# zju3dv/LoFTR

Hardware: AMD Instinct MI355X
Metric: image-pairs/sec @640x480 indoor-ds (higher is better)
Workload: dtype f32; 1 GPU; batch=8 640x480 synthetic grayscale pairs per GPU, indoor_ds dual-softmax (BASELINE configs[1]), full LoFTR.forward = ResNet-FPN backbone (HIP implicit-GEMM / patch convolutions incl. the 7x7 stem) + HIP matching path; weights=seeded random init (no checkpoint on the box), conf_matrix_materialised=True, match_type=dual_softmax, global_batch=8, parallelism=dp1 (pairs sharded; RCCL all-gather of match counts)

## Files before the change

loftr_amd/csrc/common.h:

```cpp
#pragma once
#include <hip/hip_runtime.h>
#include <stdint.h>
#include <stddef.h>
#include "../../include/loftr_hip.h"

typedef float f32x16 __attribute__((ext_vector_type(16)));
typedef float f32x4 __attribute__((ext_vector_type(4)));
typedef float f32x2 __attribute__((ext_vector_type(2)));

#define LOFTR_NEG_INF (-1e9f)

#define LOFTR_CHECK_ARG(cond) do { if (!(cond)) return LOFTR_ERR_BAD_ARG; } while (0)
#define LOFTR_CHECK_LAUNCH() do { if (hipGetLastError() != hipSuccess) return LOFTR_ERR_LAUNCH; } while (0)

#ifdef __HIP_DEVICE_COMPILE__
#define LOFTR_NO_PACKED_FP32 __attribute__((target("no-packed-fp32-ops")))
#else
#define LOFTR_NO_PACKED_FP32
#endif

__host__ __device__ static inline int ceil_div(int a, int b) { return (a + b - 1) / b; }
static inline size_t align_up(size_t x, size_t a) { return (x + a - 1) / a * a; }

enum LoftrTimedKernel {
  LOFTR_T_SCORE_STATS = 0,
  LOFTR_T_SCORE_CONF = 1,
  LOFTR_T_PROJ = 2,
  LOFTR_T_LINEAR = 3,
  LOFTR_T_LINEAR_LN = 4,
  LOFTR_T_KV = 5,
  LOFTR_T_ATTN_APPLY = 6,
  LOFTR_T_ATTN_SMALL = 7,
  LOFTR_T_GATHER = 8,
  LOFTR_T_OT_STORE = 9,
  LOFTR_T_CONV = 10,
  LOFTR_T_CONV3 = 11,
  LOFTR_T_CONV3W = 12,
  LOFTR_T_ENCODER_X = 13,
  LOFTR_T_FINE_PAIR = 14,
  LOFTR_T_COUNT = 15
};
enum LoftrDebugKey {
  LOFTR_DBG_ENCODER_SCHEDULE = 0,
  LOFTR_DBG_CONV_PERSIST_CAP,
  LOFTR_DBG_WGRAD_CHUNK,
  LOFTR_DBG_REDUCE_TALL,
  LOFTR_DBG_PCT_GRID,
  LOFTR_DBG_PCT_SKIP,
  LOFTR_DBG_PCT_QUOTA,
  LOFTR_DBG_CONV_DUO,
  LOFTR_DBG_CONV_PATCH,
  LOFTR_DBG_CONV_REM,
  LOFTR_DBG_FINE_WAVES,
  LOFTR_DBG_COUNT
};
int loftr_debug_value(int key);
extern unsigned g_loftr_timing_mask;
extern int g_loftr_range_check;
void loftr_timing_mark(int id, hipStream_t st, bool end);
struct TimedLaunch {
  int id; hipStream_t st; bool on;
  TimedLaunch(int id_, hipStream_t st_) : id(id_), st(st_), on((g_loftr_timing_mask >> id_) & 1u) {
    if (on) loftr_timing_mark(id, st, false);
  }
  ~TimedLaunch() { if (on) loftr_timing_mark(id, st, true); }
};

constexpr int NUM_XCD = 8;
static inline unsigned xcd_grid(int tiles_m, int tiles_n) { return (unsigned)(NUM_XCD * ceil_div(tiles_m, NUM_XCD) * tiles_n); }
__device__ __forceinline__ bool xcd_tile(int tiles_m, int tiles_n, int& tile_m, int& tile_n) {
  const int id = blockIdx.x, xcd = id % NUM_XCD, slot = id / NUM_XCD;
  const int chunk = ceil_div(tiles_m, NUM_XCD);
  tile_n = slot % tiles_n;
  const int local = slot / tiles_n;
  tile_m = xcd * chunk + local;
  return local < chunk && tile_m < tiles_m;
}

struct WsAlloc {
  char* base; size_t cap; size_t off;
  WsAlloc(void* p, size_t bytes) : base((char*)p), cap(bytes), off(0) {}
  template <typename T> T* take(size_t n) {
    off = align_up(off, 256);
    T* r = (T*)(base + off);
    off += n * sizeof(T);
    return r;
  }
  bool ok() const { return off <= cap; }
};

__device__ __forceinline__ float wave_sum(float v) {
#pragma unroll
  for (int o = 32; o >= 1; o >>= 1) v += __shfl_xor(v, o, 64);
  return v;
}
__device__ __forceinline__ float wave_max(float v) {
#pragma unroll
  for (int o = 32; o >= 1; o >>= 1) v = fmaxf(v, __shfl_xor(v, o, 64));
  return v;
}
#define LOFTR_DPP(v_, ctrl_) __int_as_float(__builtin_amdgcn_update_dpp(0, __float_as_int(v_), ctrl_, 0xF, 0xF, true))
#define LOFTR_DPPI(v_, ctrl_) __builtin_amdgcn_update_dpp(0, v_, ctrl_, 0xF, 0xF, true)
__device__ __forceinline__ float half_sum(float v) {
  v += LOFTR_DPP(v, 0xB1);
  v += LOFTR_DPP(v, 0x4E);
  v += LOFTR_DPP(v, 0x141);
  v += LOFTR_DPP(v, 0x140);
  const auto r = __builtin_amdgcn_permlane16_swap(__float_as_int(v), __float_as_int(v), false, false);
  return __int_as_float(r[0]) + __int_as_float(r[1]);
}
__device__ __forceinline__ float half_max(float v) {
  v = fmaxf(v, LOFTR_DPP(v, 0xB1));
  v = fmaxf(v, LOFTR_DPP(v, 0x4E));
  v = fmaxf(v, LOFTR_DPP(v, 0x141));
  v = fmaxf(v, LOFTR_DPP(v, 0x140));
  const auto r = __builtin_amdgcn_permlane16_swap(__float_as_int(v), __float_as_int(v), false, false);
  return fmaxf(__int_as_float(r[0]), __int_as_float(r[1]));
}
__device__ __forceinline__ int half_min_i32(int v) {
  v = min(v, LOFTR_DPPI(v, 0xB1));
  v = min(v, LOFTR_DPPI(v, 0x4E));
  v = min(v, LOFTR_DPPI(v, 0x141));
  v = min(v, LOFTR_DPPI(v, 0x140));
  const auto r = __builtin_amdgcn_permlane16_swap(v, v, false, false);
  return min((int)r[0], (int)r[1]);
}
__device__ __forceinline__ void half_sum16(f32x16& v) {
#pragma unroll
  for (int r = 0; r < 16; ++r) v[r] += LOFTR_DPP(v[r], 0xB1);
#pragma unroll
  for (int r = 0; r < 16; ++r) v[r] += LOFTR_DPP(v[r], 0x4E);
#pragma unroll
  for (int r = 0; r < 16; ++r) v[r] += LOFTR_DPP(v[r], 0x141);
#pragma unroll
  for (int r = 0; r < 16; ++r) v[r] += LOFTR_DPP(v[r], 0x140);
#pragma unroll
  for (int r = 0; r < 16; ++r) {
    const auto q = __builtin_amdgcn_permlane16_swap(__float_as_int(v[r]), __float_as_int(v[r]), false, false);
    v[r] = __int_as_float(q[0]) + __int_as_float(q[1]);
  }
}
__device__ __forceinline__ void half_max16(f32x16& v) {
#pragma unroll
  for (int r = 0; r < 16; ++r) v[r] = fmaxf(v[r], LOFTR_DPP(v[r], 0xB1));
#pragma unroll
  for (int r = 0; r < 16; ++r) v[r] = fmaxf(v[r], LOFTR_DPP(v[r], 0x4E));
#pragma unroll
  for (int r = 0; r < 16; ++r) v[r] = fmaxf(v[r], LOFTR_DPP(v[r], 0x141));
#pragma unroll
  for (int r = 0; r < 16; ++r) v[r] = fmaxf(v[r], LOFTR_DPP(v[r], 0x140));
#pragma unroll
  for (int r = 0; r < 16; ++r) {
    const auto q = __builtin_amdgcn_permlane16_swap(__float_as_int(v[r]), __float_as_int(v[r]), false, false);
    v[r] = fmaxf(__int_as_float(q[0]), __int_as_float(q[1]));
  }
}
__device__ __forceinline__ float swap32(float v) {
  const auto r = __builtin_amdgcn_permlane32_swap(__float_as_int(v), __float_as_int(v), false, false);
  return __int_as_float((threadIdx.x & 32) ? r[0] : r[1]);
}
#define LOFTR_DPP_SWAP32(v_) swap32(v_)

__device__ __forceinline__ float elu1(float x) {
  return x > 0.f ? x + 1.f : __expf(x);
}
```

loftr_amd/csrc/conv.hip:

```cpp
#include "gemm.h"
#include "conv_prepared.h"
#include <stdlib.h>

namespace {

using CfgD = GemmCfg<256, 128, 4, 2, 3>;

struct ConvArgs {
  ASrc a;
  const sp_t* w; int K;
  const float* bias;
  const float* wscale;
  const float* x_inv;
  const sp_t* residual;
  sp_t* y_sp;
  float* y_f32;
  int M, Cout, Coutp;
  int act;
  const sp_t* up;
  int Hl, Wl;
  float sy, sx;
};

template <typename Cfg, bool FULL>
// ... 266 lines not shown
        acc[i][j] = __builtin_amdgcn_mfma_f32_32x32x16_f16(fh[(R0_) + i][ks_], bl[ks_][j], acc[i][j], 0, 0, 0); \
    _Pragma("unroll") for (int i = 0; i < 2; ++i)                                                           \
      _Pragma("unroll") for (int j = 0; j < (NJ_); ++j)                                                     \
        acc[i][j] = __builtin_amdgcn_mfma_f32_32x32x16_f16(fh[(R0_) + i][ks_], bh[ks_][j], acc[i][j], 0, 0, 0); \
  }
#define C3_PIN_PAIRS(n_)                                                                                    \
    _Pragma("unroll") for (int u__ = 0; u__ < (n_); ++u__) {                                                \
      __builtin_amdgcn_sched_group_barrier(0x008, 1, 0);                                                    \
      __builtin_amdgcn_sched_group_barrier(0x100, 1, 0);                                                    \
    }
#define C3_ITER(KY, NJ_, DEAD_)                                                                             \
  {                                                                                                         \
    const int tt__ = t + (KY);                                                                              \
     \
    const int newer__ = (tt__ + 2 < nk ? 2 : 0) + ((patch_m1 || patch_m2) ? PQ : 0);                        \
    if (newer__ >= 2 + PQ) LOFTR_WAITCNT_VM(2 + PQ);                                                        \
    else if (newer__ >= PQ) LOFTR_WAITCNT_VM(PQ);                                                           \
    else if (newer__ >= 2) LOFTR_WAITCNT_VM(2);                                                             \
    else LOFTR_WAITCNT_VM(0);                                                                               \
    __builtin_amdgcn_s_barrier();                                                                           \
    if (tt__ + 3 < nk) C3_ISSUE_B(cg3, (q3 % 3) * 3 + q3 / 3, (bstage + 3) & 3);                            \
    if (++q3 == 9) { q3 = 0; ++cg3; }                                                                       \
    patch_m2 = patch_m1;                                                                                    \
    patch_m1 = false;                                                                                       \
    if ((KY) == 0 && kx == 0 && cg + 1 < gpt) { C3_ISSUE_PATCH(cg + 1, (cg + 1) & 1); patch_m1 = true; }    \
    if ((NJ_) > 0) {                                                                                        \
      constexpr int n1__ = ((KY) == 0 ? 4 : 2) + 2 * (NJ_);                 \
      constexpr int n0__ = ((KY) == 2 ? 4 : 2) + 2 * (NJ_);             \
      if (!(DEAD_)) {                                                                                       \
        if ((KY) == 0) { C3_LOAD_ROW(0, 1, sP, kx); C3_LOAD_ROW(1, 1, sP, kx); }                            \
        else C3_LOAD_ROW((KY) + 1, 1, sP, kx);                                                              \
        C3_LOAD_B(1, bstage, NJ_);                                                                          \
      }                                                                                                     \
      C3_MFMAS(0, KY, NJ_);                                                                                 \
                                         \
      if ((KY) == 2) { C3_LOAD_ROW(0, 0, sPn, kxn); C3_LOAD_ROW(1, 0, sPn, kxn); }                          \
      else C3_LOAD_ROW((KY) + 2, 0, sP, kx);                                                                \
      C3_LOAD_B(0, (bstage + 1) & 3, NJ_);                                                                  \
      if (!(DEAD_)) C3_MFMAS(1, KY, NJ_);                                                                   \
                            \
      if (!(DEAD_)) {                                                                                       \
        C3_PIN_PAIRS(n1__) __builtin_amdgcn_sched_group_barrier(0x008, 6 * (NJ_) - n1__, 0);                \
      }                                                                                                     \
      C3_PIN_PAIRS(n0__) __builtin_amdgcn_sched_group_barrier(0x008, 6 * (NJ_) - n0__, 0);                  \
    }                                                                                                       \
    bstage = (bstage + 1) & 3;                                                                              \
  }
#define C3_TRIP(NJ_, DEAD_)                                                                                 \
  {                                                                                                         \
    const char* sP = patch_base + (cg & 1) * PATCH_BYTES;                                                   \
    const int kxn = kx == 2 ? 0 : kx + 1;                           \
    const char* sPn = patch_base + ((cg + (kx == 2 ? 1 : 0)) & 1) * PATCH_BYTES;                            \
    C3_ITER(0, NJ_, DEAD_)                                                                                  \
    C3_ITER(1, NJ_, DEAD_)                                                                                  \
    C3_ITER(2, NJ_, DEAD_)                                                                                  \
    if (++kx == 3) { kx = 0; ++cg; }                                                                        \
  }
  const bool dead_last = p.Cin <= (gpt - 1) * 32 + 16;
#define C3_LOOP(NJ_)                                                                                        \
  {                                                                                                         \
     \
    LOFTR_WAITCNT_VM(4);                                                                                    \
    __builtin_amdgcn_s_barrier();                                                                           \
    if ((NJ_) > 0) {                                                                                        \
      C3_LOAD_ROW(0, 0, patch_base, 0);                                                                     \
      C3_LOAD_ROW(1, 0, patch_base, 0);                                                                     \
      C3_LOAD_B(0, 0, NJ_);                                                                                 \
    }                                                                                                       \
    int t = 0;                                                                                              \
    for (; t < nk - 9; t += 3) C3_TRIP(NJ_, 0)                                                              \
    if (dead_last) { for (; t < nk; t += 3) C3_TRIP(NJ_, 1) }                                               \
    else { for (; t < nk; t += 3) C3_TRIP(NJ_, 0) }                                                         \
  }
  if (nact == 2) C3_LOOP(2)
  else if (nact == 1) C3_LOOP(1)
  else C3_LOOP(0)
#undef C3_LOOP
#undef C3_TRIP
#undef C3_ITER
#undef C3_PIN_PAIRS
#undef C3_MFMAS
#undef C3_LOAD_B
#undef C3_LOAD_ROW

  vid += gridDim.x;
  C3_NEXT_TILE()
  __builtin_amdgcn_s_barrier();
  if (have) {
    C3_DMA_OFFSETS()
    C3_ISSUE_PATCH(0, 0);
    C3_ISSUE_B(0, 0, 0);
    C3_ISSUE_B(0, 3, 1);
    C3_ISSUE_B(0, 6, 2);
  }

  const bool odd = lane & 1;
  const int Ho = p.H, Wo = p.W;
#pragma unroll
  for (int j = 0; j < 2; ++j) {
    const int col = n0 + wn * 64 + j * 32 + tx;
    const bool creal = col < p.Cout, cpad = col < p.Coutp;
    const float bia = (p.bias && creal) ? p.bias[col] : 0.f;
    const float wsc = (creal ? p.wscale[col] : 1.f) * (p.x_inv ? *p.x_inv : 1.f);
    const int spc = (col & ~31) + (odd ? 16 : 0) + ((col & 31) >> 1);
#pragma unroll
    for (int i = 0; i < 2; ++i) {
      const int y = y0 + wm * 2 + i;
      f32x16 v = acc[i][j] * wsc;
      uint32_t rw[16];
      if (p.residual) {
#pragma unroll
        for (int r = 0; r < 16; ++r) {
          const int x = x0 + (r & 3) + 8 * (r >> 2) + 4 * g;
          const bool ok = y < Ho && x < Wo && cpad;
          rw[r] = ok ? p.residual[(unsigned)(((b * Ho + y) * Wo + x) * p.Coutp + spc)] : 0u;
        }
#pragma unroll
        for (int r = 0; r < 16; ++r) v[r] += sp_value(rw[r], odd);
      }
#pragma unroll
      for (int r = 0; r < 16; ++r) {
        float xv = v[r] + bia;
        if (p.act == 1) xv = fmaxf(xv, 0.f);
        if (p.act == 2) xv = xv > 0.f ? xv : 0.01f * xv;
        v[r] = creal ? xv : 0.f;
      }
      if (p.y_f32) {
#pragma unroll
        for (int r = 0; r < 16; ++r) {
          const int x = x0 + (r & 3) + 8 * (r >> 2) + 4 * g;
          if (y < Ho && x < Wo && creal) p.y_f32[(unsigned)(((b * Ho + y) * Wo + x) * p.Cout + col)] = v[r];
        }
      }
      if (p.y_sp) {
        uint32_t w16[16];
        sp_words16(v, odd, w16);
#pragma unroll
        for (int r = 0; r < 16; ++r) {
          const int x = x0 + (r & 3) + 8 * (r >> 2) + 4 * g;
          if (y < Ho && x < Wo && cpad) p.y_sp[(unsigned)(((b * Ho + y) * Wo + x) * p.Coutp + spc)] = w16[r];
        }
      }
    }
  }
  if (!have) break;
  }
#undef C3_ISSUE_PATCH
#undef C3_ISSUE_B
#undef C3_DMA_OFFSETS
#undef C3_NEXT_TILE
}

#include "conv3x3_duo.h"


__global__ __launch_bounds__(256) void conv_rowscale_kernel(const float* __restrict__ w, const float* __restrict__ bn_w,
                                                            const float* __restrict__ bn_b, const float* __restrict__ bn_m,
                                                            const float* __restrict__ bn_v, float eps, int Cin, int KH, int KW,
                                                            long s_co, long s_ci, long s_ky, long s_kx,
                                                            float* __restrict__ bias, float* __restrict__ wscale) {
  const int co = blockIdx.x;
  float scale = 1.f, shift = 0.f;
  if (bn_w) {
    scale = bn_w[co] / sqrtf(bn_v[co] + eps);
    shift = bn_b[co] - bn_m[co] * scale;
  }
  float m = 0.f;
  for (int t = threadIdx.x; t < Cin * KH * KW; t += 256) {
    const int c = t % Cin, tap = t / Cin;
    m = fmaxf(m, fabsf(w[co * s_co + c * s_ci + (tap / KW) * s_ky + (tap % KW) * s_kx] * scale));
  }
  __shared__ float red[4];
  m = wave_max(m);
  if ((threadIdx.x & 63) == 0) red[threadIdx.x >> 6] = m;
  __syncthreads();
  if (threadIdx.x == 0) {
    float inv;
    (void)sp_row_scale(fmaxf(fmaxf(red[0], red[1]), fmaxf(red[2], red[3])), &inv);
    bias[co] = shift;
    wscale[co] = inv;
  }
}

__global__ __launch_bounds__(256) void conv_prep_kernel(const float* __restrict__ w, const float* __restrict__ bn_w,
                                                        const float* __restrict__ bn_b, const float* __restrict__ bn_m,
                                                        const float* __restrict__ bn_v, float eps, int Cin, int Cp,
                                                        int KH, int KW, long s_co, long s_ci, long s_ky, long s_kx,
                                                        sp_t* __restrict__ wsp, const float* __restrict__ wscale) {
  const int co = blockIdx.y;
  const int K = KH * KW * Cp;
  float scale = 1.f;
  if (bn_w) scale = bn_w[co] / sqrtf(bn_v[co] + eps);
  const float up = 1.f / wscale[co];
  const int grp = blockIdx.x * 8 + (threadIdx.x >> 5);
  if (grp * 32 >= K) return;
  const int col = grp * 32 + (threadIdx.x & 31);
  const int tap = col / Cp, c = col - tap * Cp;
  float v = 0.f;
  if (c < Cin) v = (w[co * s_co + c * s_ci + (tap / KW) * s_ky + (tap % KW) * s_kx] * scale) * up;
  sp_store(wsp + (long)co * K, col, v, true);
}

__global__ __launch_bounds__(256) void upsample_add_kernel(const sp_t* __restrict__ low, const sp_t* __restrict__ lat,
                                                           sp_t* __restrict__ out, int Hl, int Wl, int Cp, long nitems) {
  const long item = (long)blockIdx.x * 256 + threadIdx.x;
  if (item >= nitems) return;
  const int octs = Cp >> 3;
  const long pix = item / octs;
  const int oct = (int)(item - pix * octs);
  const int Ho = 2 * Hl, Wo = 2 * Wl;
  const int x = (int)(pix % Wo), y = (int)((pix / Wo) % Ho);
  const long b = pix / ((long)Wo * Ho);
  const float sy = Ho > 1 ? (float)(Hl - 1) / (float)(Ho - 1) : 0.f, sx = Wo > 1 ? (float)(Wl - 1) / (float)(Wo - 1) : 0.f;
  const float fy = sy * (float)y, fx = sx * (float)x;
  const int y0 = (int)fy, x0 = (int)fx;
  const int y1 = y0 + (y0 < Hl - 1 ? 1 : 0), x1 = x0 + (x0 < Wl - 1 ? 1 : 0);
  const float ly = fy - (float)y0, lx = fx - (float)x0;
  const float hy = 1.f - ly, hx = 1.f - lx;
  const int off = sp_octet_off(oct);
  const sp_t* src[5] = {low + ((b * Hl + y0) * Wl + x0) * Cp + off, low + ((b * Hl + y0) * Wl + x1) * Cp + off,
                        low + ((b * Hl + y1) * Wl + x0) * Cp + off, low + ((b * Hl + y1) * Wl + x1) * Cp + off,
                        lat + pix * Cp + off};
  u32x4 hi[5], lo[5];
#pragma unroll
  for (int t = 0; t < 5; ++t) {
    hi[t] = *reinterpret_cast<const u32x4*>(src[t]);
    lo[t] = *reinterpret_cast<const u32x4*>(src[t] + 16);
  }
  float v[5][8];
#pragma unroll
  for (int t = 0; t < 5; ++t) sp_unpack8(hi[t], lo[t], v[t]);
  float r[8];
#pragma unroll
  for (int e = 0; e < 8; ++e)
    r[e] = v[4][e] + (hy * (hx * v[0][e] + lx * v[1][e]) + ly * (hx * v[2][e] + lx * v[3][e]));
  u32x4 oh, ol;
  sp_pack8(r, oh, ol);
  sp_t* o = out + pix * Cp + off;
  *reinterpret_cast<u32x4*>(o) = oh;
  *reinterpret_cast<u32x4*>(o + 16) = ol;
}

constexpr int STEM_TY = 8, STEM_TX = 32;
__global__ __launch_bounds__(256) void stem_conv_kernel(const float* __restrict__ x, long sxb, long sxh, long sxw,
                                                        int H, int W, const float* __restrict__ w, long s_co, long s_ky,
                                                        long s_kx, const float* __restrict__ bn_w,
                                                        const float* __restrict__ bn_b, const float* __restrict__ bn_m,
                                                        const float* __restrict__ bn_v, float eps, int C0, int Ho, int Wo,
                                                        sp_t* __restrict__ y) {
  constexpr int IH = 2 * STEM_TY + 5, IW = 2 * STEM_TX + 5;
  __shared__ float tile[IH][IW + 3];
  const int b = blockIdx.z, oy0 = blockIdx.y * STEM_TY, ox0 = blockIdx.x * STEM_TX;
  const float* xb = x + (long)b * sxb;
  for (int e = threadIdx.x; e < IH * IW; e += 256) {
    const int r = e / IW, c = e - r * IW;
    const int iy = 2 * oy0 - 3 + r, ix = 2 * ox0 - 3 + c;
    tile[r][c] = ((unsigned)iy < (unsigned)H && (unsigned)ix < (unsigned)W) ? xb[iy * sxh + ix * sxw] : 0.f;
  }
  const int ch = threadIdx.x & 127, slot = threadIdx.x >> 7;
  float wr[49];
  float scale = 1.f, shift = 0.f;
  if (ch < C0) {
    if (bn_w) { scale = bn_w[ch] / sqrtf(bn_v[ch] + eps); shift = bn_b[ch] - bn_m[ch] * scale; }
#pragma unroll
    for (int t = 0; t < 49; ++t) wr[t] = w[ch * s_co + (t / 7) * s_ky + (t % 7) * s_kx] * scale;
  } else {
#pragma unroll
    for (int t = 0; t < 49; ++t) wr[t] = 0.f;
  }
  __syncthreads();
  const int Cp = (C0 + 31) / 32 * 32;
  for (int q = slot; q < STEM_TY * STEM_TX / 4; q += 2) {
    const int py = q / (STEM_TX / 4), px = (q - py * (STEM_TX / 4)) * 4;
    float acc[4] = {shift, shift, shift, shift};
#pragma unroll
    for (int ky = 0; ky < 7; ++ky) {
      float row[13];
#pragma unroll
      for (int c = 0; c < 13; ++c) row[c] = tile[2 * py + ky][2 * px + c];
#pragma unroll
      for (int kx = 0; kx < 7; ++kx)
#pragma unroll
        for (int e = 0; e < 4; ++e) acc[e] += row[2 * e + kx] * wr[ky * 7 + kx];
    }
    const int oy = oy0 + py;
#pragma unroll
    for (int e = 0; e < 4; ++e) {
      const int ox = ox0 + px + e;
      const float v = fmaxf(acc[e], 0.f);
      const bool ok = oy < Ho && ox < Wo && ch < Cp;
      const uint32_t word = sp_word(ch < C0 ? v : 0.f, ch & 1);
      if (ok) y[(((long)b * Ho + oy) * Wo + ox) * Cp + sp_index(ch)] = word;
    }
  }
}

__global__ void sp_to_f32_kernel(const sp_t* __restrict__ src, float* __restrict__ dst, long rows, int C, int Cp) {
  const long row = blockIdx.x;
  for (int c = threadIdx.x; c < Cp; c += blockDim.x) {
    const float v = sp_value(src[row * Cp + sp_index(c)], c & 1);
    if (c < C) dst[row * C + c] = v;
  }
}

}

extern "C" size_t loftr_conv_workspace_bytes(int Cin, int Cout, int KH, int KW) {
  if (Cin <= 0 || Cout <= 0 || KH <= 0 || KW <= 0) return 0;
  return align_up((size_t)Cout * KH * KW * ceil32(Cin) * 4, 256) + 2 * align_up((size_t)Cout * 4, 256) + 2048;
}

static unsigned persistent_grid(unsigned nvirt) {
  const int cap = loftr_debug_value(LOFTR_DBG_CONV_PERSIST_CAP);
  const int forced = cap >= NUM_XCD ? cap / NUM_XCD * NUM_XCD : -1;
  int cus = forced;
  if (cus < 0) {
    static int per_dev[64];
    int dev = 0, n = 0;
    if (hipGetDevice(&dev) != hipSuccess || dev < 0 || dev >= 64) return nvirt;
    if (per_dev[dev] == 0) {
      if (hipDeviceGetAttribute(&n, hipDeviceAttributeMultiprocessorCount, dev) != hipSuccess) return nvirt;
      per_dev[dev] = n / NUM_XCD * NUM_XCD;
    }
    cus = per_dev[dev];
  }
  return cus > 0 && nvirt > (unsigned)cus ? (unsigned)cus : nvirt;
}

template <int RT>
__global__ __launch_bounds__(256) void conv_rem_gather_kernel(const float* __restrict__ pbuf, long npix, int H, int W, int R, int c0, int Coutp,
                                                              const float* __restrict__ bias, const sp_t* __restrict__ residual, int act,
                                                              sp_t* __restrict__ y_sp) {
  const long pix = (long)blockIdx.x * 256 + threadIdx.x;
  if (pix >= npix) return;
  const int x = (int)(pix % W), y = (int)((pix / W) % H);
  float v[8];
#pragma unroll
  for (int c = 0; c < 8; ++c) v[c] = 0.f;
  const float* pp = pbuf + pix * (9 * R);
#pragma unroll
  for (int ky = 0; ky < 3; ++ky)
#pragma unroll
    for (int kx = 0; kx < 3; ++kx) {
      const int yy = y + ky - 1, xx = x + kx - 1;
      if ((unsigned)yy < (unsigned)H && (unsigned)xx < (unsigned)W) {
        const float* q = pp + ((long)(ky - 1) * W + (kx - 1)) * (9 * R) + (ky * 3 + kx) * R;
        if (RT == 4) {
          const f32x4 t = *reinterpret_cast<const f32x4*>(q);
          v[0] += t[0]; v[1] += t[1]; v[2] += t[2]; v[3] += t[3];
        } else {
#pragma unroll
          for (int c = 0; c < 7; ++c) if (c < R) v[c] += q[c];
        }
      }
    }
  sp_t* row = y_sp + pix * Coutp + c0;
  float rv[8];
#pragma unroll
  for (int c = 0; c < 8; ++c) rv[c] = 0.f;
  if (residual) {
    const sp_t* rr = residual + pix * Coutp + c0;
    const u32x4 hi = *reinterpret_cast<const u32x4*>(rr), lo = *reinterpret_cast<const u32x4*>(rr + 16);
    sp_unpack8(hi, lo, rv);
  }
  const float slope = act == 1 ? 0.f : act == 2 ? 0.01f : 1.f;
  float o[8];
#pragma unroll
  for (int c = 0; c < 8; ++c) {
    const float t = v[c] + ((bias && c < R) ? bias[c0 + c] : 0.f) + rv[c];
    o[c] = c < R ? fmaxf(t, slope * t) : 0.f;
  }
  u32x4 oh, ol;
  sp_pack8(o, oh, ol);
  const u32x4 z = {0u, 0u, 0u, 0u};
  u32x4* dst = reinterpret_cast<u32x4*>(row);
  dst[0] = oh; dst[1] = z; dst[2] = z; dst[3] = z; dst[4] = ol; dst[5] = z; dst[6] = z; dst[7] = z;
}


static int conv_prepare(const float* weight, const long* weight_strides, int Cin, int Cout, int KH, int KW,
                        const float* bn_weight, const float* bn_bias, const float* bn_mean, const float* bn_var, float bn_eps,
                        void* buf, size_t bytes, hipStream_t st) {
  LOFTR_CHECK_ARG(weight && weight_strides && buf && Cin > 0 && Cout > 0 && KH > 0 && KW > 0);
  LOFTR_CHECK_ARG((bn_weight == nullptr) == (bn_bias == nullptr) && (bn_weight == nullptr) == (bn_mean == nullptr) &&
                  (bn_weight == nullptr) == (bn_var == nullptr));
  ConvPrepared pr;
  if (!conv_prepared_layout(buf, bytes, Cin, Cout, KH, KW, pr)) return LOFTR_ERR_WORKSPACE;
  const int Cp = ceil32(Cin), K = KH * KW * Cp;
  (void)hipMemsetAsync(pr.zeros, 0, 256, st);
  hipLaunchKernelGGL(conv_rowscale_kernel, dim3(Cout), dim3(256), 0, st, weight, bn_weight, bn_bias, bn_mean, bn_var, bn_eps,
                     Cin, KH, KW, weight_strides[0], weight_strides[1], weight_strides[2], weight_strides[3], pr.bias, pr.wscale);
  hipLaunchKernelGGL(conv_prep_kernel, dim3(ceil_div(K / 32, 8), Cout), dim3(256), 0, st, weight, bn_weight, bn_bias,
                     bn_mean, bn_var, bn_eps, Cin, Cp, KH, KW, weight_strides[0], weight_strides[1], weight_strides[2],
                     weight_strides[3], pr.wsp, pr.wscale);
  LOFTR_CHECK_LAUNCH();
  return LOFTR_OK;
}

static int conv_rem_channels(int Cout, int KH, int KW, int stride) {
  return (KH == 3 && KW == 3 && stride == 1 && ceil32(Cout) == 224 && Cout - 192 >= 1 && Cout - 192 <= 7) ? Cout - 192 : 0;
}
extern "C" size_t loftr_conv_scratch_bytes(int B, int H, int W, int Cout, int KH, int KW, int stride) {
  const int R = conv_rem_channels(Cout, KH, KW, stride);
  return (R > 0 && B > 0 && H > 0 && W > 0) ? (size_t)B * H * W * 9 * R * 4 : 0;
}

static int conv_run(const uint32_t* x_sp, int B, int H, int W, int Cin, const void* prepared, size_t prepared_bytes, int Cout,
                    int KH, int KW, int stride, int pad, int act, const uint32_t* residual_sp, const uint32_t* up_sp,
                    uint32_t* y_sp, float* y_f32, void* stream, const float* x_inv = nullptr, void* scratch = nullptr, size_t scratch_bytes = 0) {
  LOFTR_CHECK_ARG(x_sp && prepared && (y_sp || y_f32) && B >= 0 && H > 0 && W > 0 && Cin > 0 && Cout > 0);
  const bool shared_gpu = (act & LOFTR_CONV_SHARED_GPU) != 0;
  act &= ~LOFTR_CONV_SHARED_GPU;
  LOFTR_CHECK_ARG(KH > 0 && KW > 0 && stride > 0 && pad >= 0 && act >= 0 && act <= 2);
  if (B == 0) return LOFTR_OK;
  hipStream_t st = (hipStream_t)stream;
  ConvGeom g;
  g.H = H; g.W = W; g.Cp = ceil32(Cin); g.KH = KH; g.KW = KW; g.stride = stride; g.pad = pad;
  g.Ho = (H + 2 * pad - KH) / stride + 1;
  g.Wo = (W + 2 * pad - KW) / stride + 1;
  if (g.Ho <= 0 || g.Wo <= 0 || H >= 32768 || W >= 32768) return LOFTR_ERR_UNSUPPORTED;
  if (up_sp && ((g.Ho & 1) || (g.Wo & 1) || KH != 1 || KW != 1 || stride != 1 || pad != 0 || !y_sp || y_f32 || residual_sp || act != 0))
    return LOFTR_ERR_UNSUPPORTED;
  const long M = (long)B * g.Ho * g.Wo;
  if (M * (long)ceil32(Cout) >= (1L << 31) || (long)B * H * W * g.Cp >= (1L << 31)) return LOFTR_ERR_UNSUPPORTED;
  const int K = KH * KW * g.Cp;
  ConvPrepared pr;
  if (!conv_prepared_layout(const_cast<void*>(prepared), prepared_bytes, Cin, Cout, KH, KW, pr)) return LOFTR_ERR_WORKSPACE;
  sp_t* wsp = pr.wsp;
  float* bias = pr.bias;
  sp_t* zeros = pr.zeros;
  g.zeros = zeros;
  ConvArgs p;
  p.a = asrc_conv(x_sp, g);
  p.w = wsp; p.K = K; p.bias = bias; p.wscale = pr.wscale; p.x_inv = x_inv; p.residual = residual_sp; p.y_sp = y_sp; p.y_f32 = y_f32;
  p.M = (int)M; p.Cout = Cout; p.Coutp = ceil32(Cout); p.act = act;
  p.up = up_sp; p.Hl = g.Ho / 2; p.Wl = g.Wo / 2;
  p.sy = g.Ho > 1 ? (float)(p.Hl - 1) / (float)(g.Ho - 1) : 0.f;
  p.sx = g.Wo > 1 ? (float)(p.Wl - 1) / (float)(g.Wo - 1) : 0.f;
  if (loftr_debug_value(LOFTR_DBG_CONV_PATCH) && KH == 3 && KW == 3 && stride == 1 && pad == 1 && !up_sp) {
    Conv3Args c;
    c.x = x_sp; c.B = B; c.H = H; c.W = W; c.Cp = g.Cp; c.Cin = Cin; c.w = wsp; c.K = K; c.bias = bias; c.wscale = pr.wscale; c.x_inv = x_inv; c.residual = residual_sp;
    c.y_sp = y_sp; c.y_f32 = y_f32; c.Cout = Cout; c.Coutp = ceil32(Cout); c.act = act; c.zeros = zeros;
    c.tiles_x = ceil_div(W, c3::TX); c.tiles_y = ceil_div(H, c3::TY); c.pbuf = nullptr;
    const bool duo = loftr_debug_value(LOFTR_DBG_CONV_DUO) != 0;
    const bool wide = duo && c.Coutp == 32 * 7;
    TimedLaunch tl(wide ? LOFTR_T_CONV3W : LOFTR_T_CONV3, st);
    if (duo && c.Coutp % 128 == 0) {
      using CF = c3d::Cfg<4, 2, 4>;
      c.tiles_y = ceil_div(H, CF::TY);
      hipLaunchKernelGGL((conv3x3_duo_kernel<CF>), dim3(xcd_grid(B * c.tiles_x * c.tiles_y, c.Coutp / 128)), dim3(256), 0, st, c);
    } else if (duo && c.Coutp == 192) {
      using CF = c3d::Cfg<6, 2, 4, 8, 2>;
      c.tiles_y = ceil_div(H, CF::TY);
      hipLaunchKernelGGL((conv3x3_duo_kernel<CF>), dim3(xcd_grid(B * c.tiles_x * c.tiles_y, 1)), dim3(512), 0, st, c);
    } else if (wide && conv_rem_channels(Cout, KH, KW, stride) > 0 && !y_f32 && loftr_debug_value(LOFTR_DBG_CONV_REM) &&
               scratch && scratch_bytes >= (size_t)B * H * W * 9 * conv_rem_channels(Cout, KH, KW, stride) * 4) {
      using CF = c3d::Cfg<6, 2, 4, 8, 2, true>;
      c.tiles_y = ceil_div(H, CF::TY);
      c.pbuf = reinterpret_cast<float*>(scratch);
      hipLaunchKernelGGL((conv3x3_duo_kernel<CF>), dim3(xcd_grid(B * c.tiles_x * c.tiles_y, 1)), dim3(512), 0, st, c);
      LOFTR_CHECK_LAUNCH();
      const long npix = (long)B * H * W;
      if (Cout - 192 == 4)
        hipLaunchKernelGGL(conv_rem_gather_kernel<4>, dim3((unsigned)((npix + 255) / 256)), dim3(256), 0, st, c.pbuf, npix, H, W, 4, 192, c.Coutp,
                           bias, residual_sp, act, y_sp);
      else
        hipLaunchKernelGGL(conv_rem_gather_kernel<0>, dim3((unsigned)((npix + 255) / 256)), dim3(256), 0, st, c.pbuf, npix, H, W, Cout - 192, 192, c.Coutp,
                           bias, residual_sp, act, y_sp);
    } else if (wide) {
      using CF = c3d::Cfg<7, 2, 4, 8, 2>;
      c.tiles_y = ceil_div(H, CF::TY);
      hipLaunchKernelGGL((conv3x3_duo_kernel<CF>), dim3(xcd_grid(B * c.tiles_x * c.tiles_y, 1)), dim3(512), 0, st, c);
    } else
      hipLaunchKernelGGL(conv3x3_kernel, dim3(shared_gpu ? xcd_grid(B * c.tiles_x * c.tiles_y, ceil_div(c.Coutp, 128))
                                                         : persistent_grid(xcd_grid(B * c.tiles_x * c.tiles_y, ceil_div(c.Coutp, 128)))),
                         dim3(512), 0, st, c);
    LOFTR_CHECK_LAUNCH();
    return LOFTR_OK;
  }
  {
    TimedLaunch tl(LOFTR_T_CONV, st);
    if (up_sp)
      hipLaunchKernelGGL((conv_kernel<CfgD, true>), dim3(xcd_grid(ceil_div(p.M, CfgD::BM), ceil_div(p.Coutp, CfgD::BN))),
                         dim3(CfgD::THREADS), 0, st, p);
    else
      hipLaunchKernelGGL((conv_kernel<CfgD, false>), dim3(xcd_grid(ceil_div(p.M, CfgD::BM), ceil_div(p.Coutp, CfgD::BN))),
                         dim3(CfgD::THREADS), 0, st, p);
  }
  LOFTR_CHECK_LAUNCH();
  return LOFTR_OK;
}

#ifdef LOFTR_CONV_PROBE
extern "C" int loftr_conv_probe_buffer(void* buf) {
  long long* b = (long long*)buf;
  return hipMemcpyToSymbol(HIP_SYMBOL(g_conv_probe), &b, sizeof(b)) == hipSuccess ? LOFTR_OK : LOFTR_ERR_LAUNCH;
}
#endif

extern "C" int loftr_conv_prepare(const float* weight, const long* weight_strides, int Cin, int Cout, int KH, int KW,
                                  const float* bn_weight, const float* bn_bias, const float* bn_mean, const float* bn_var,
                                  float bn_eps, void* prepared, size_t prepared_bytes, void* stream) {
  return conv_prepare(weight, weight_strides, Cin, Cout, KH, KW, bn_weight, bn_bias, bn_mean, bn_var, bn_eps, prepared,
                      prepared_bytes, (hipStream_t)stream);
}

extern "C" int loftr_conv_bn_act_prepared(const uint32_t* x_sp, int B, int H, int W, int Cin, const void* prepared,
                                          size_t prepared_bytes, int Cout, int KH, int KW, int stride, int pad, int act,
                                          const uint32_t* residual_sp, const uint32_t* low_sp, uint32_t* y_sp, float* y_f32,
                                          const float* x_inv_scale, void* stream) {
  return conv_run(x_sp, B, H, W, Cin, prepared, prepared_bytes, Cout, KH, KW, stride, pad, act, residual_sp, low_sp, y_sp, y_f32,
                  stream, x_inv_scale);
}

extern "C" int loftr_conv_bn_act_prepared_scratch(const uint32_t* x_sp, int B, int H, int W, int Cin, const void* prepared,
                                                  size_t prepared_bytes, int Cout, int KH, int KW, int stride, int pad, int act,
                                                  const uint32_t* residual_sp, const uint32_t* low_sp, uint32_t* y_sp, float* y_f32,
                                                  const float* x_inv_scale, void* scratch, size_t scratch_bytes, void* stream) {
  return conv_run(x_sp, B, H, W, Cin, prepared, prepared_bytes, Cout, KH, KW, stride, pad, act, residual_sp, low_sp, y_sp, y_f32,
                  stream, x_inv_scale, scratch, scratch_bytes);
}

extern "C" int loftr_conv_bn_act(const uint32_t* x_sp, int B, int H, int W, int Cin, const float* weight,
                                 const long* weight_strides, int Cout, int KH, int KW, int stride, int pad, const float* bn_weight, const float* bn_bias,
                                 const float* bn_mean, const float* bn_var, float bn_eps, int act,
                                 const uint32_t* residual_sp, uint32_t* y_sp, float* y_f32, void* ws, size_t ws_bytes,
                                 const float* x_inv_scale, void* stream) {
  LOFTR_CHECK_ARG(x_sp && (y_sp || y_f32) && B >= 0 && H > 0 && W > 0);
  if (B == 0) return LOFTR_OK;
  const int rc = conv_prepare(weight, weight_strides, Cin, Cout, KH, KW, bn_weight, bn_bias, bn_mean, bn_var, bn_eps, ws, ws_bytes,
                              (hipStream_t)stream);
  if (rc != LOFTR_OK) return rc;
  return conv_run(x_sp, B, H, W, Cin, ws, ws_bytes, Cout, KH, KW, stride, pad, act, residual_sp, nullptr, y_sp, y_f32, stream, x_inv_scale);
}

extern "C" int loftr_conv1x1_upsample_add(const uint32_t* x_sp, int B, int H, int W, int Cin, const float* weight,
                                          const long* weight_strides, int Cout, const uint32_t* low_sp, uint32_t* y_sp,
                                          void* ws, size_t ws_bytes, void* stream) {
  LOFTR_CHECK_ARG(x_sp && low_sp && y_sp && B >= 0 && H > 0 && W > 0);
  if (B == 0) return LOFTR_OK;
  const int rc = conv_prepare(weight, weight_strides, Cin, Cout, 1, 1, nullptr, nullptr, nullptr, nullptr, 0.f, ws, ws_bytes,
                              (hipStream_t)stream);
  if (rc != LOFTR_OK) return rc;
  return conv_run(x_sp, B, H, W, Cin, ws, ws_bytes, Cout, 1, 1, 1, 0, 0, nullptr, low_sp, y_sp, nullptr, stream);
}

extern "C" int loftr_stem_conv_bn_relu(const float* x, const long* x_strides, int B, int H, int W, const float* weight,
                                       const long* weight_strides, int C0, const float* bn_weight, const float* bn_bias,
                                       const float* bn_mean, const float* bn_var, float bn_eps, uint32_t* y_sp,
                                       void* stream) {
  LOFTR_CHECK_ARG(x && x_strides && weight && weight_strides && y_sp && B >= 0 && H > 0 && W > 0 && C0 > 0);
  LOFTR_CHECK_ARG((bn_weight == nullptr) == (bn_bias == nullptr) && (bn_weight == nullptr) == (bn_mean == nullptr) &&
                  (bn_weight == nullptr) == (bn_var == nullptr));
  if (C0 > 128) return LOFTR_ERR_UNSUPPORTED;
  if (B == 0) return LOFTR_OK;
  const int Ho = (H + 6 - 7) / 2 + 1, Wo = (W + 6 - 7) / 2 + 1;
  hipLaunchKernelGGL(stem_conv_kernel, dim3(ceil_div(Wo, STEM_TX), ceil_div(Ho, STEM_TY), B), dim3(256), 0,
                     (hipStream_t)stream, x, x_strides[0], x_strides[2], x_strides[3], H, W, weight, weight_strides[0],
                     weight_strides[2], weight_strides[3], bn_weight, bn_bias, bn_mean, bn_var, bn_eps, C0, Ho, Wo, y_sp);
  LOFTR_CHECK_LAUNCH();
  return LOFTR_OK;
}

extern "C" int loftr_upsample2x_add(const uint32_t* low_sp, const uint32_t* lateral_sp, uint32_t* out_sp, int B, int Hl,
                                    int Wl, int C, void* stream) {
  LOFTR_CHECK_ARG(low_sp && lateral_sp && out_sp && B >= 0 && Hl > 0 && Wl > 0 && C > 0);
  if (B == 0) return LOFTR_OK;
  const int Cp = ceil32(C);
  const long pixels = (long)B * 4 * Hl * Wl;
  if (pixels >= (1L << 31)) return LOFTR_ERR_UNSUPPORTED;
  const long nitems = pixels * (Cp / 8);
  if ((nitems + 255) / 256 >= (1L << 31)) return LOFTR_ERR_UNSUPPORTED;
  hipLaunchKernelGGL(upsample_add_kernel, dim3((unsigned)((nitems + 255) / 256)), dim3(256), 0, (hipStream_t)stream,
                     low_sp, lateral_sp, out_sp, Hl, Wl, Cp, nitems);
  LOFTR_CHECK_LAUNCH();
  return LOFTR_OK;
}

extern "C" int loftr_sp_from_f32(const float* src, uint32_t* dst_sp, long rows, int C, void* stream) {
  LOFTR_CHECK_ARG(src && dst_sp && rows >= 0 && C > 0);
  return launch_sp_convert1(src, C, dst_sp, rows, C, (hipStream_t)stream);
}

extern "C" int loftr_sp_from_f32_scaled(const float* src, uint32_t* dst_sp, long rows, int C, float* inv_scale_out, void* stream) {
  LOFTR_CHECK_ARG(src && dst_sp && inv_scale_out && rows >= 0 && C > 0);
  return launch_sp_convert1(src, C, dst_sp, rows, C, (hipStream_t)stream, inv_scale_out);
}

extern "C" int loftr_sp_to_f32(const uint32_t* src_sp, float* dst, long rows, int C, void* stream) {
  LOFTR_CHECK_ARG(src_sp && dst && rows >= 0 && C > 0);
  if (rows == 0) return LOFTR_OK;
  const int Cp = ceil32(C);
  hipLaunchKernelGGL(sp_to_f32_kernel, dim3((unsigned)rows), dim3(Cp > 256 ? 256 : Cp), 0, (hipStream_t)stream, src_sp,
                     dst, rows, C, Cp);
  LOFTR_CHECK_LAUNCH();
  return LOFTR_OK;
}
```

loftr_amd/csrc/misc.hip:

```cpp
#include "common.h"
#include <string.h>

namespace {
template <bool CL>
__global__ void pos_encode_flatten_kernel(loftr_fmap f, const float* __restrict__ pe,
                                          int pe_h, int pe_w, float* __restrict__ out, int C) {
  __shared__ float tile[32][33];
  const int H = f.H, W = f.W, HW = H * W;
  const int n = blockIdx.z, hw0 = blockIdx.x * 32, c0 = blockIdx.y * 32;
  const float* in = f.data + (long)n * f.sn;
  for (int k = threadIdx.y; k < 32; k += 8) {
    const int c = c0 + k, hw = hw0 + threadIdx.x;
    float v = 0.f;
    if (c < C && hw < HW) {
      const int y = hw / W, x = hw - y * W;
      v = pe[((long)c * pe_h + y) * pe_w + x];
      if (!CL) v += in[(long)c * f.sc + (long)y * f.sh + (long)x * f.sw];
    }
    tile[k][threadIdx.x] = v;
  }
  __syncthreads();
  for (int k = threadIdx.y; k < 32; k += 8) {
    const int hw = hw0 + k, c = c0 + threadIdx.x;
    if (hw < HW && c < C) {
      float v = tile[threadIdx.x][k];
      if (CL) { const int y = hw / W, x = hw - y * W; v += in[(long)y * f.sh + (long)x * f.sw + c]; }
      out[((long)n * HW + hw) * C + c] = v;
    }
  }
}
}

extern "C" int loftr_pos_encode_flatten(const loftr_fmap* feat, const float* pe, int pe_h, int pe_w, float* out,
                                        int N, int C, void* stream) {
  LOFTR_CHECK_ARG(feat && feat->data && pe && out && N >= 0 && C > 0 && feat->H > 0 && feat->W > 0 &&
                  feat->H <= pe_h && feat->W <= pe_w);
  if (N == 0) return LOFTR_OK;
  const dim3 grid(ceil_div(feat->H * feat->W, 32), ceil_div(C, 32), N), block(32, 8);
  if (feat->sc == 1)
    hipLaunchKernelGGL((pos_encode_flatten_kernel<true>), grid, block, 0, (hipStream_t)stream, *feat, pe, pe_h, pe_w, out, C);
  else
    hipLaunchKernelGGL((pos_encode_flatten_kernel<false>), grid, block, 0, (hipStream_t)stream, *feat, pe, pe_h, pe_w, out, C);
  LOFTR_CHECK_LAUNCH();
  return LOFTR_OK;
}

namespace {
struct DebugSwitch { const char* name; int def; int value; };
DebugSwitch g_debug[LOFTR_DBG_COUNT] = {{"encoder_schedule", 1, 1}, {"conv_persist_cap", 0, 0}, {"wgrad_chunk", 0, 0}, {"reduce_tall", 1, 1},
                                        {"pct_grid", 0, 0}, {"pct_skip", 0, 0}, {"pct_quota", 0, 0}, {"conv_duo", 1, 1}, {"conv_patch", 1, 1}, {"conv_rem", 1, 1},
                                        {"fine_waves", 0, 0}};
}
int loftr_debug_value(int key) { return (key >= 0 && key < LOFTR_DBG_COUNT) ? g_debug[key].value : 0; }
extern "C" int loftr_hip_debug_set(const char* key, int value) {
  LOFTR_CHECK_ARG(key != nullptr);
  for (auto& d : g_debug)
    if (strcmp(d.name, key) == 0) { d.value = value; return LOFTR_OK; }
  return LOFTR_ERR_BAD_ARG;
}
extern "C" int loftr_hip_debug_get(const char* key, int* value, int* default_value) {
  LOFTR_CHECK_ARG(key != nullptr && value != nullptr);
  for (auto& d : g_debug)
    if (strcmp(d.name, key) == 0) { *value = d.value; if (default_value) *default_value = d.def; return LOFTR_OK; }
  return LOFTR_ERR_BAD_ARG;
}

unsigned g_loftr_timing_mask = 0;
int g_loftr_range_check = 0;
extern "C" int loftr_hip_range_check_enable(int on) { g_loftr_range_check = on ? 1 : 0; return LOFTR_OK; }
namespace {
constexpr int T_POOL = 4096;
struct TimingSlot {
  hipEvent_t ev[T_POOL][2];
  int created, used;
  double total_ms; long long launches;
};
TimingSlot g_slots[LOFTR_T_COUNT];
const char* const T_NAMES[LOFTR_T_COUNT] = {"score_sweep_kernel<0>", "score_sweep_kernel<1>", "proj_kernel", "linear_kernel",
                                            "linear_ln_kernel", "proj_kv_kernel", "attn_apply_kernel",
                                            "attn_small_kernel", "gather_windows_kernel", "score_sweep_kernel<2>", "conv_kernel",
                                            "conv3x3_duo_kernel<Cfg<4,2,4,4,1>>", "conv3x3_duo_kernel<Cfg<7,2,4,8,2>>", "encoder_x_kernel", "fine_pair_kernel"};
void timing_drain(TimingSlot& s) {
  for (int i = 0; i < s.used; ++i) {
    float ms = 0.f;
    if (hipEventSynchronize(s.ev[i][1]) == hipSuccess && hipEventElapsedTime(&ms, s.ev[i][0], s.ev[i][1]) == hipSuccess) {
      s.total_ms += ms;
      s.launches += 1;
    }
  }
  s.used = 0;
}
}

void loftr_timing_mark(int id, hipStream_t st, bool end) {
  TimingSlot& s = g_slots[id];
  if (!end) {
    if (s.used >= T_POOL) return;
    if (s.used >= s.created) {
      if (hipEventCreate(&s.ev[s.created][0]) != hipSuccess || hipEventCreate(&s.ev[s.created][1]) != hipSuccess) return;
      s.created++;
    }
    (void)hipEventRecord(s.ev[s.used][0], st);
  } else {
    if (s.used >= s.created) return;
    (void)hipEventRecord(s.ev[s.used][1], st);
    s.used++;
  }
}

extern "C" int loftr_hip_timing_enable(unsigned mask) {
  g_loftr_timing_mask = mask & ((1u << LOFTR_T_COUNT) - 1u);
  return LOFTR_OK;
}

extern "C" int loftr_hip_timing_kernel_count(void) { return LOFTR_T_COUNT; }

extern "C" const char* loftr_hip_timing_kernel_name(int id) {
  return (id >= 0 && id < LOFTR_T_COUNT) ? T_NAMES[id] : "";
}

extern "C" int loftr_hip_timing_read(int id, double* total_ms, long long* launches, int reset) {
  LOFTR_CHECK_ARG(id >= 0 && id < LOFTR_T_COUNT && total_ms && launches);
  TimingSlot& s = g_slots[id];
  timing_drain(s);
  *total_ms = s.total_ms;
  *launches = s.launches;
  if (reset) { s.total_ms = 0.0; s.launches = 0; }
  return LOFTR_OK;
}

extern "C" int loftr_hip_abi_version(void) { return LOFTR_HIP_ABI_VERSION; }

extern "C" const char* loftr_hip_status_string(int status) {
  switch (status) {
    case LOFTR_OK: return "ok";
    case LOFTR_ERR_BAD_ARG: return "bad argument (null pointer or invalid shape)";
    case LOFTR_ERR_UNSUPPORTED: return "shape not supported by the gfx950 kernels";
    case LOFTR_ERR_WORKSPACE: return "workspace too small";
    case LOFTR_ERR_LAUNCH: return "HIP kernel launch failed";
    case LOFTR_ERR_NO_DEVICE: return "no gfx950 (MI355X) device";
    case LOFTR_ERR_COMM: return "RCCL unavailable or a communicator / collective call failed";
    case LOFTR_ERR_RANGE: return "an activation entering the split-fp16 GEMM chain is not below the fp16 maximum 65504 (or not finite)";
    default: return "unknown status";
  }
}

extern "C" int loftr_hip_device_check(void) {
  int dev = 0;
  if (hipGetDevice(&dev) != hipSuccess) return LOFTR_ERR_NO_DEVICE;
  hipDeviceProp_t prop;
  if (hipGetDeviceProperties(&prop, dev) != hipSuccess) return LOFTR_ERR_NO_DEVICE;
  return strncmp(prop.gcnArchName, "gfx950", 6) == 0 ? LOFTR_OK : LOFTR_ERR_NO_DEVICE;
}
```

Measured before the change: 457.3 image-pairs/s.

## Add full-width-N conv entry kernel for 224/256-channel implicit-GEMM convolutions

Adds a new implicit-GEMM convolution kernel that covers the whole output-channel width (224 or 256) in one 512-thread block, with a 4-stage LDS ring fed by global_load_lds and split-fp16 MFMA. It is selected by default, behind a heuristic that checks whether the tile count fills the CUs well enough. Covering all output channels in one block means each input activation tile is loaded once rather than once per N tile. In exchange the kernel uses large LDS, runs one block per CU, and issues fewer, larger tiles, which can hurt occupancy on layers with a small M.

Result: no change. 459.5 image-pairs/s (median of 5 runs) (+0.5%).

```diff
diff --git a/loftr_amd/csrc/common.h b/loftr_amd/csrc/common.h
--- a/loftr_amd/csrc/common.h
+++ b/loftr_amd/csrc/common.h
@@ -52,6 +52,7 @@
   LOFTR_DBG_CONV_PATCH,
   LOFTR_DBG_CONV_REM,
   LOFTR_DBG_FINE_WAVES,
+  LOFTR_DBG_CONV_ENTRY,
   LOFTR_DBG_COUNT
 };
 int loftr_debug_value(int key);
diff --git a/loftr_amd/csrc/conv.hip b/loftr_amd/csrc/conv.hip
--- a/loftr_amd/csrc/conv.hip
+++ b/loftr_amd/csrc/conv.hip
@@ -442,6 +442,7 @@
 }
 
 #include "conv3x3_duo.h"
+#include "conv_entry.h"
 
 
 __global__ __launch_bounds__(256) void conv_rowscale_kernel(const float* __restrict__ w, const float* __restrict__ bn_w,
@@ -693,6 +694,17 @@
 extern "C" size_t loftr_conv_scratch_bytes(int B, int H, int W, int Cout, int KH, int KW, int stride) {
   const int R = conv_rem_channels(Cout, KH, KW, stride);
   return (R > 0 && B > 0 && H > 0 && W > 0) ? (size_t)B * H * W * 9 * R * 4 : 0;
+}
+
+template <typename CF>
+static void conv_entry_launch(const ConvArgs& p, hipStream_t st) {
+  hipLaunchKernelGGL((entry_tile_kernel<CF>), dim3(xcd_grid(ceil_div(p.M, CF::BM), 1)), dim3(CF::THREADS), 0, st, p);
+}
+static bool conv_entry_pays(int M) {
+  const int cus = (int)persistent_grid(1u << 30);
+  if (cus <= 0 || cus >= (1 << 30)) return false;
+  const int tiles = ceil_div(M, 256), rounds = ceil_div(tiles, cus);
+  return 4 * tiles >= 3 * rounds * cus;
 }
 
 static int conv_run(const uint32_t* x_sp, int B, int H, int W, int Cin, const void* prepared, size_t prepared_bytes, int Cout,
@@ -770,7 +782,11 @@
   }
   {
     TimedLaunch tl(LOFTR_T_CONV, st);
-    if (up_sp)
+    const int entry = up_sp ? 0 : loftr_debug_value(LOFTR_DBG_CONV_ENTRY);
+    if (entry && (p.Coutp == 224 || p.Coutp == 256) && (entry == 2 || conv_entry_pays(p.M))) {
+      if (p.Coutp == 224) conv_entry_launch<ce::Cfg<2, 7>>(p, st);
+      else conv_entry_launch<ce::Cfg<2, 8>>(p, st);
+    } else if (up_sp)
       hipLaunchKernelGGL((conv_kernel<CfgD, true>), dim3(xcd_grid(ceil_div(p.M, CfgD::BM), ceil_div(p.Coutp, CfgD::BN))),
                          dim3(CfgD::THREADS), 0, st, p);
     else
diff --git a/loftr_amd/csrc/conv_entry.h b/loftr_amd/csrc/conv_entry.h
--- /dev/null
+++ b/loftr_amd/csrc/conv_entry.h
@@ -0,0 +1,165 @@
+#pragma once
+
+namespace ce {
+template <int TM_, int NT_>
+struct Cfg {
+  static constexpr int TM = TM_, TN = 4, NT = NT_, WM = 4, WN = 2, WAVES = 8, THREADS = 512, NS = 4;
+  static constexpr int WTM = TM * 32, WTN = TN * 32, BM = WM * WTM, BN = WN * WTN;
+  static constexpr int A_SLOTS = BM / 16, B_SLOTS = NT * 2;
+  static constexpr int AQ = A_SLOTS / WAVES, BQ = (B_SLOTS + WAVES - 1) / WAVES, PER = AQ + BQ;
+  static constexpr int A_BYTES = A_SLOTS * 1024, STAGE_BYTES = (A_SLOTS + B_SLOTS) * 1024;
+  static constexpr int LDS_BYTES = NS * STAGE_BYTES + 1024;
+  static_assert(A_SLOTS % WAVES == 0 && NT > TN && NT <= 2 * TN, "DMA mapping; two wave splits of 4 and NT - 4 column tiles");
+  static_assert(LDS_BYTES <= 160 * 1024, "LDS");
+};
+}
+
+template <typename CF>
+__device__ __forceinline__ void conv_entry_mainloop(const ConvArgs& p, int m0, char* lds, f32x16 (&acc)[CF::TM][CF::TN]) {
+  constexpr int TM = CF::TM, TN = CF::TN, NS = CF::NS, AQ = CF::AQ, BQ = CF::BQ, PER = CF::PER, WAVES = CF::WAVES;
+  typedef __attribute__((address_space(3))) void* lds_ptr_t;
+  typedef const __attribute__((address_space(1))) void* gbl_ptr_t;
+  const ConvGeom& cv = p.a.cv;
+  const int tid = threadIdx.x, lane = tid & 63, wave = tid >> 6;
+  const int wm = wave % CF::WM, wn = wave / CF::WM;
+  const int g = lane >> 5, tx = lane & 31;
+  const int drow = lane >> 2, dpos = lane & 3;
+  char* const scratch = lds + NS * CF::STAGE_BYTES;
+
+  int aoff[AQ], ayx[AQ], boff[BQ];
+#pragma unroll
+  for (int q = 0; q < AQ; ++q) {
+    const int r = (q * WAVES + wave) * 16 + drow;
+    const int c = dpos ^ ((r >> 2) & 3);
+    const int gr = min(m0 + r, p.M - 1);
+    const int hw = cv.Ho * cv.Wo;
+    const int b = gr / hw, rem = gr - b * hw;
+    const int yo = rem / cv.Wo, xo = rem - yo * cv.Wo;
+    const int yb = yo * cv.stride - cv.pad, xb = xo * cv.stride - cv.pad;
+    ayx[q] = (yb << 16) | (xb & 0xffff);
+    aoff[q] = ((b * cv.H + yb) * cv.W + xb) * cv.Cp + (((c & 1) + ((c >> 1) << 2)) << 2);
+  }
+#pragma unroll
+  for (int q = 0; q < BQ; ++q) {
+    const int r = (q * WAVES + wave) * 16 + drow;
+    const int c = dpos ^ ((r >> 2) & 3);
+    boff[q] = min(r, p.Cout - 1) * p.K + (((c & 1) + ((c >> 1) << 2)) << 2);
+  }
+  const int gpt = cv.Cp >> 5, ns = 2 * cv.KH * cv.KW * gpt;
+  int is_h = 0, is_cg = 0, is_ky = 0, is_kx = 0, is_toff = 0, is_k0 = 0;
+
+#define CE_WAITCNT_VM_LGKM0(n_) __builtin_amdgcn_s_waitcnt((((n_) & 0xF) | (((n_) >> 4) << 14) | (0x7 << 4)))
+#define CE_ISSUE(stage_)                                                                                    \
+  {                                                                                                         \
+    char* s__ = lds + (stage_) * CF::STAGE_BYTES;                                                           \
+    _Pragma("unroll") for (int q = 0; q < AQ; ++q) {                                                        \
+      const int y__ = (ayx[q] >> 16) + is_ky, x__ = (int)(short)(ayx[q] & 0xffff) + is_kx;                  \
+      const bool in__ = (unsigned)y__ < (unsigned)cv.H && (unsigned)x__ < (unsigned)cv.W;                   \
+      const sp_t* g__ = in__ ? p.a.p0 + (aoff[q] + is_toff) : cv.zeros;                                     \
+      __builtin_amdgcn_global_load_lds((gbl_ptr_t)g__, (lds_ptr_t)(s__ + (q * WAVES + wave) * 1024), 16, 0, 0); \
+    }                                                                                                       \
+    _Pragma("unroll") for (int q = 0; q < BQ; ++q) {                                                        \
+      char* d__ = (q * WAVES + wave < CF::B_SLOTS) ? s__ + CF::A_BYTES + (q * WAVES + wave) * 1024 : scratch; \
+      __builtin_amdgcn_global_load_lds((gbl_ptr_t)(p.w + (boff[q] + is_k0)), (lds_ptr_t)d__, 16, 0, 0);     \
+    }                                                                                                       \
+    is_toff += 8; is_k0 += 8;                                              \
+    if ((is_h ^= 1) == 0) {                                                                                 \
+      is_toff += 16; is_k0 += 16;                                 \
+      if (++is_cg == gpt) {                                                                                 \
+        is_cg = 0;                                                \
+        if (++is_kx == cv.KW) { is_kx = 0; ++is_ky; is_toff += (cv.W - cv.KW) * cv.Cp; }                    \
+      }                                                                                                     \
+    }                                                                                                       \
+  }
+
+  int abase[TM], bbase[TN];
+#pragma unroll
+  for (int i = 0; i < TM; ++i) {
+    const int ar = wm * CF::WTM + i * 32 + tx;
+    abase[i] = ar * 64 + ((g ^ ((ar >> 2) & 3)) << 4);
+  }
+#pragma unroll
+  for (int j = 0; j < TN; ++j) {
+    const int br = min(wn * TN + j, CF::NT - 1) * 32 + tx;
+    bbase[j] = CF::A_BYTES + br * 64 + ((g ^ ((br >> 2) & 3)) << 4);
+  }
+#define CE_READ(ah_, al_, bh_, bl_, stage_, NJ_)                                                            \
+  {                                                                                                         \
+    const char* s__ = lds + (stage_) * CF::STAGE_BYTES;                                                     \
+    _Pragma("unroll") for (int i = 0; i < TM; ++i) {                                                        \
+      ah_[i] = *reinterpret_cast<const h16x8*>(s__ + abase[i]);                                             \
+      al_[i] = *reinterpret_cast<const h16x8*>(s__ + (abase[i] ^ 32));                                      \
+    }                                                                                                       \
+    _Pragma("unroll") for (int j = 0; j < (NJ_); ++j) {                                                     \
+      bh_[j] = *reinterpret_cast<const h16x8*>(s__ + bbase[j]);                                             \
+      bl_[j] = *reinterpret_cast<const h16x8*>(s__ + (bbase[j] ^ 32));                                      \
+    }                                                                                                       \
+  }
+#define CE_STEP(s_, ah_, al_, bh_, bl_, nah_, nal_, nbh_, nbl_, NJ_)                                        \
+  {                                                                                                         \
+     \
+    if ((s_) + 2 < ns) CE_WAITCNT_VM_LGKM0(PER);                                                            \
+    else CE_WAITCNT_VM_LGKM0(0);                                                                            \
+    __builtin_amdgcn_s_barrier();             \
+    if ((s_) + NS - 1 < ns) CE_ISSUE(((s_) + NS - 1) & (NS - 1));                                           \
+    CE_READ(nah_, nal_, nbh_, nbl_, ((s_) + 1) & (NS - 1), NJ_);      \
+    _Pragma("unroll") for (int i = 0; i < TM; ++i)                                                          \
+      _Pragma("unroll") for (int j = 0; j < (NJ_); ++j)                                                     \
+        acc[i][j] = __builtin_amdgcn_mfma_f32_32x32x16_f16(al_[i], bh_[j], acc[i][j], 0, 0, 0);             \
+    _Pragma("unroll") for (int i = 0; i < TM; ++i)                                                          \
+      _Pragma("unroll") for (int j = 0; j < (NJ_); ++j)                                                     \
+        acc[i][j] = __builtin_amdgcn_mfma_f32_32x32x16_f16(ah_[i], bl_[j], acc[i][j], 0, 0, 0);             \
+    _Pragma("unroll") for (int i = 0; i < TM; ++i)                                                          \
+      _Pragma("unroll") for (int j = 0; j < (NJ_); ++j)                                                     \
+        acc[i][j] = __builtin_amdgcn_mfma_f32_32x32x16_f16(ah_[i], bh_[j], acc[i][j], 0, 0, 0);             \
+                            \
+    _Pragma("unroll") for (int u__ = 0; u__ < 2 * TM + 2 * (NJ_); ++u__) {                                  \
+      __builtin_amdgcn_sched_group_barrier(0x008, 1, 0);                                                    \
+      __builtin_amdgcn_sched_group_barrier(0x100, 1, 0);                                                    \
+    }                                                                                                       \
+    __builtin_amdgcn_sched_group_barrier(0x008, 3 * TM * (NJ_) - 2 * TM - 2 * (NJ_), 0);                    \
+  }
+
+#pragma unroll
+  for (int i = 0; i < TM; ++i)
+#pragma unroll
+    for (int j = 0; j < TN; ++j)
+#pragma unroll
+      for (int r = 0; r < 16; ++r) acc[i][j][r] = 0.f;
+
+  static_assert(NS == 4, "ring indices are masked; the waits below leave one step in flight");
+#pragma unroll
+  for (int s = 0; s < NS - 1; ++s)
+    if (s < ns) CE_ISSUE(s);
+  if (ns > 2) LOFTR_WAITCNT_VM(2 * PER);
+  else LOFTR_WAITCNT_VM(PER);
+  __builtin_amdgcn_s_barrier();
+  h16x8 ah0[TM], al0[TM], bh0[TN], bl0[TN], ah1[TM], al1[TM], bh1[TN], bl1[TN];
+#define CE_LOOP(NJ_)                                                                                        \
+  {                                                                                                         \
+    CE_READ(ah0, al0, bh0, bl0, 0, NJ_);                                                                    \
+    for (int s = 0; s < ns; s += 2) {                                                                       \
+      CE_STEP(s, ah0, al0, bh0, bl0, ah1, al1, bh1, bl1, NJ_)                                               \
+      CE_STEP(s + 1, ah1, al1, bh1, bl1, ah0, al0, bh0, bl0, NJ_)                                           \
+    }                                                                                                       \
+  }
+  if (CF::NT == 2 * TN || wn == 0) CE_LOOP(TN)
+  else CE_LOOP(CF::NT - TN)
+#undef CE_LOOP
+#undef CE_STEP
+#undef CE_READ
+#undef CE_ISSUE
+#undef CE_WAITCNT_VM_LGKM0
+}
+
+template <typename CF>
+__global__ __launch_bounds__(CF::THREADS, 1) void entry_tile_kernel(ConvArgs p) {
+  __shared__ __attribute__((aligned(16))) char lds[CF::LDS_BYTES];
+  int tm, tn;
+  if (!xcd_tile(ceil_div(p.M, CF::BM), 1, tm, tn)) return;
+  const int m0 = tm * CF::BM;
+  f32x16 acc[CF::TM][CF::TN];
+  conv_entry_mainloop<CF>(p, m0, lds, acc);
+  if (m0 + CF::BM <= p.M) conv_epilogue<CF, true>(p, acc, m0, 0);
+  else conv_epilogue<CF, false>(p, acc, m0, 0);
+}
diff --git a/loftr_amd/csrc/misc.hip b/loftr_amd/csrc/misc.hip
--- a/loftr_amd/csrc/misc.hip
+++ b/loftr_amd/csrc/misc.hip
@@ -49,7 +49,7 @@
 struct DebugSwitch { const char* name; int def; int value; };
 DebugSwitch g_debug[LOFTR_DBG_COUNT] = {{"encoder_schedule", 1, 1}, {"conv_persist_cap", 0, 0}, {"wgrad_chunk", 0, 0}, {"reduce_tall", 1, 1},
                                         {"pct_grid", 0, 0}, {"pct_skip", 0, 0}, {"pct_quota", 0, 0}, {"conv_duo", 1, 1}, {"conv_patch", 1, 1}, {"conv_rem", 1, 1},
-                                        {"fine_waves", 0, 0}};
+                                        {"fine_waves", 0, 0}, {"conv_entry", 1, 1}};
 }
 int loftr_debug_value(int key) { return (key >= 0 && key < LOFTR_DBG_COUNT) ? g_debug[key].value : 0; }
 extern "C" int loftr_hip_debug_set(const char* key, int value) {
```
